# ssheybani/baby-vision-curriculum

Measured on AMD Instinct MI355X. Metric: video clips/sec (node) VideoMAE-base 16x224^2 bf16 pretraining, higher is better.
Workload: dtype bf16

## Files before the change

### __graft_entry__.py

```python
import importlib.util
import os
import subprocess
import sys

ROOT = os.path.dirname(os.path.abspath(__file__))
PKG_DIR = os.path.join(ROOT, "baby-vision-curriculum_amd")
CSRC = os.path.join(PKG_DIR, "csrc")
LIB = os.path.join(PKG_DIR, "libbvc_hip.so")
PRODUCT_SOURCES = ["gemm.hip", "gemm_persist.hip", "gemm8.hip", "gemm_as.hip", "attention.hip", "rowops.hip", "stack.hip", "videomae.hip", "jepa.hip", "comm.hip"]
EXPERIMENT_SOURCES = [os.path.join("experiments", "gemm_big.hip"), os.path.join("experiments", "gemm_pp.hip")]
EXPERIMENT_INCLUDES = [os.path.join("experiments", "attention_dq_wave96.inc")]
HEADERS = ["common.h", "gemm.h", "gemm_tile.h", "attention.h", "rowops.h", "stack.h", os.path.join("..", "..", "include", "bvc.h")]


def _experiments():
    return "BVC_EXPERIMENTS" in os.environ.get("BVC_EXTRA_HIPCC_FLAGS", "")


def _sources():
    return PRODUCT_SOURCES + (EXPERIMENT_SOURCES if _experiments() else [])


SOURCES = PRODUCT_SOURCES


EXPERIMENT_FLAGS = {"attention.hip": ["-mllvm", "-amdgpu-mfma-vgpr-form=1"]}


def _extra_flags(src):
    return EXPERIMENT_FLAGS.get(src, []) if _experiments() else []


HASH_FILE = LIB + ".srchash"


def _source_hash():
    import hashlib
    h = hashlib.sha256()
    for f in _sources() + HEADERS + (EXPERIMENT_INCLUDES if _experiments() else []):
        with open(os.path.join(CSRC, f), "rb") as fh:
            h.update(f.encode() + b"\0" + fh.read())
    h.update(os.environ.get("BVC_EXTRA_HIPCC_FLAGS", "").encode())
    return h.hexdigest()


def _stale():
    if not (os.path.exists(LIB) and os.path.exists(HASH_FILE)):
        return True
    with open(HASH_FILE) as fh:
        return fh.read().strip() != _source_hash()


def _hash_of(files):
# ... 98 lines not shown
```

### baby-vision-curriculum_amd/_lib.py

```python
import ctypes
import os

_HERE = os.path.dirname(os.path.abspath(__file__))
LIB_PATH = os.environ.get("BVC_LIB_PATH") or os.path.join(_HERE, "libbvc_hip.so")

c_void_p, c_int, c_int64, c_float, c_char_p = ctypes.c_void_p, ctypes.c_int, ctypes.c_int64, ctypes.c_float, ctypes.c_char_p
c_double = ctypes.c_double


class BvcError(RuntimeError):
    pass


class VideoMAEConfigC(ctypes.Structure):
    _fields_ = [(n, c_int) for n in (
        "image_size", "patch_size", "num_channels", "num_frames", "tubelet_size",
        "hidden_size", "num_hidden_layers", "num_attention_heads", "intermediate_size",
        "decoder_hidden_size", "decoder_num_hidden_layers", "decoder_num_attention_heads",
        "decoder_intermediate_size")] + [("layer_norm_eps", c_float), ("decoder_norm_eps", c_float),
                                         ("norm_pix_loss", c_int)]


class VitConfigC(ctypes.Structure):
    _fields_ = [(n, c_int) for n in ("image_size", "patch_size", "num_channels", "num_frames", "tubelet_size", "embed_dim",
# ... 110 lines not shown
    "bvc_op_gemm_plan_dw": (c_int, [ctypes.POINTER(GemmDesc), c_int]),
    "bvc_op_attention_fwd": (c_int, [c_void_p, c_void_p, c_void_p, c_int, c_int, c_int, c_int, c_void_p]),
    "bvc_op_attention_bwd": (c_int, [c_void_p, c_void_p, c_void_p, c_void_p, c_void_p, c_void_p, c_int, c_int, c_int, c_int, c_void_p]),
    "bvc_op_attention_bwd_part": (c_int, [c_void_p, c_void_p, c_void_p, c_void_p, c_void_p, c_void_p, c_int, c_int, c_int, c_int, c_int, c_void_p]),
    "bvc_op_layernorm_fwd": (c_int, [c_void_p, c_int, c_int, c_int, c_void_p, c_void_p, c_void_p, c_void_p, c_void_p,
                                     c_int, c_int, c_float, c_void_p]),
    "bvc_op_layernorm_bwd": (c_int, [c_void_p, c_void_p, c_int, c_int, c_int, c_void_p, c_void_p, c_void_p, c_void_p,
                                     c_int, c_void_p, c_void_p, c_void_p, c_void_p, c_int, c_int, c_void_p]),
    "bvc_op_layernorm_bwd_workspace": (c_int64, [c_int, c_int]),
    "bvc_op_colsum_bf16": (c_int, [c_void_p, c_int, c_int, c_int, c_float, c_void_p, c_void_p, c_void_p]),
    "bvc_op_cast_bf16": (c_int, [c_void_p, c_void_p, c_int64, c_void_p]),
    "bvc_op_row_normalize": (c_int, [c_void_p, c_void_p, c_void_p, c_int, c_int, c_float, c_void_p]),
    "bvc_op_row_normalize_bwd": (c_int, [c_void_p, c_void_p, c_void_p, c_void_p, c_int, c_int, c_void_p]),
    "bvc_op_nce_finalize": (c_int, [c_void_p, c_int, c_float, c_int64, c_void_p, c_void_p, c_void_p]),
    "bvc_op_sgd_step": (c_int, [c_void_p, c_void_p, c_void_p, c_int64, c_float, c_float, c_float, c_float, c_int, c_int, c_int,
                                c_void_p, c_void_p, c_int, c_void_p, c_void_p]),
    "bvc_videomae_shadow": (c_int, [c_void_p, c_int, ctypes.POINTER(c_void_p), ctypes.POINTER(c_int64)]),
    "bvc_vit_shadow": (c_int, [c_void_p, c_int, ctypes.POINTER(c_void_p), ctypes.POINTER(c_int64)]),
    "bvc_predictor_shadow": (c_int, [c_void_p, c_int, ctypes.POINTER(c_void_p), ctypes.POINTER(c_int64)]),
    "bvc_op_adam_prepare": (c_int, [c_void_p, c_double, c_double, c_double, c_void_p, c_void_p]),
    "bvc_op_adam_step": (c_int, [c_void_p, c_void_p, c_void_p, c_void_p, c_int64, c_double, c_double, c_double, c_double, c_double,
                                 c_int, c_int, c_void_p, c_void_p, c_void_p, c_int, c_void_p, c_void_p]),
    "bvc_op_row_ln_selected": (c_int, [c_int, c_int, c_int, c_int]),
    "bvc_op_sgd_step_segments": (c_int, [c_void_p, c_void_p, c_void_p, c_int64, c_void_p, c_void_p, c_void_p, c_int, c_void_p, c_void_p, c_void_p,
                                         c_int, c_void_p, c_void_p]),
    "bvc_op_adam_step_segments": (c_int, [c_void_p, c_void_p, c_void_p, c_void_p, c_int64, c_void_p, c_void_p, c_void_p, c_int, c_void_p, c_void_p,
                                          c_void_p, c_void_p, c_void_p, c_int, c_void_p, c_void_p]),
    "bvc_op_nonfinite_check": (c_int, [c_void_p, c_int64, c_void_p, c_void_p]),
    "bvc_op_mask_index": (c_int, [c_void_p, c_int, c_int, c_int, c_int, c_void_p, c_void_p, c_void_p, c_void_p]),
    "bvc_op_gather_patches": (c_int, [c_void_p, c_void_p, c_void_p, c_int, c_int, c_int, c_int, c_int, c_int, c_int, c_int, c_void_p]),
    "bvc_op_pixel_labels": (c_int, [c_void_p, c_void_p, c_void_p, c_int, c_int, c_int, c_int, c_int, c_int, c_int, c_int, c_int, c_void_p]),
    "bvc_comm_unique_id": (c_int, [c_void_p]),
    "bvc_comm_init": (c_int, [c_int, c_int, c_void_p, ctypes.POINTER(c_void_p)]),
    "bvc_comm_destroy": (c_int, [c_void_p]),
    "bvc_comm_stream": (c_void_p, [c_void_p]),
    "bvc_comm_rank": (c_int, [c_void_p]),
    "bvc_comm_world": (c_int, [c_void_p]),
    "bvc_comm_library": (c_char_p, []),
    "bvc_allreduce_bucket": (c_int, [c_void_p, c_void_p, c_int64, c_int, c_void_p]),
    "bvc_comm_wait": (c_int, [c_void_p, c_void_p]),
    "bvc_allgather": (c_int, [c_void_p, c_void_p, c_void_p, c_int64, c_void_p]),
    "bvc_allreduce": (c_int, [c_void_p, c_void_p, c_int64, c_int, c_void_p]),
    "bvc_broadcast": (c_int, [c_void_p, c_void_p, c_int64, c_int, c_void_p]),
}

_lib = None
# ... 33 lines not shown
```

### baby-vision-curriculum_amd/csrc/attention.h

```cpp
#pragma once
#include "common.h"

namespace bvc {
int launch_attn_fwd(const bf16_t* qkv, bf16_t* ctx, float* lse, int B, int N, int H, int head_dim, hipStream_t stream,
                    float softmax_scale = 0.f);
int launch_attn_bwd(const bf16_t* qkv, const bf16_t* ctx, const bf16_t* dctx, const float* lse, float* delta,
                    bf16_t* dqkv, int B, int N, int H, int head_dim, hipStream_t stream, float softmax_scale = 0.f, int parts = 3);
}
```

### baby-vision-curriculum_amd/csrc/attention.hip

```cpp
#include <stdlib.h>

#include "attention.h"

namespace bvc {

#define AS3 __attribute__((address_space(3)))
#define MFMA32(a, b, c) __builtin_amdgcn_mfma_f32_32x32x16_bf16((a), (b), (c), 0, 0, 0)

template <int HD>
__device__ __forceinline__ int swz_dual(int r) {
    if constexpr (HD == 64) return (((r >> 1) & 1) << 2) | ((r >> 2) & 3);
    else return (r >> 2) & 3;
}

template <int HD, int NW = 4>
__device__ __forceinline__ void stage64(__amdgpu_buffer_rsrc_t rs, int row0, int ld, int col0, char* lds,
                                        int wave, int lane) {
    constexpr int CPR = HD / 8;
    constexpr int RPP = 64 / CPR;
#pragma unroll
    for (int jj = 0; jj < (HD / 8 + NW - 1) / NW; ++jj) {
        const int j = wave + NW * jj;
        if (NW > HD / 8 && j >= HD / 8) break;
        const int r = RPP * j + lane / CPR;
        const int c = (lane % CPR) ^ swz_dual<HD>(r);
// ... 115 lines not shown
        s[r] = fast_exp2(fmaf(s[r], scale_log2, nm));
        rs += s[r];
    }
    st.l_run += rs;
    const bf16x8 p0 = acc_to_frag(s, 0), p1 = acc_to_frag(s, 1);
#pragma unroll
    for (int t = 0; t < HD / 32; ++t) st.o[t] = MFMA32(lds_tr<VOFF>(lds, fa.tr[t][0], fa.tr[t][1]), p0, st.o[t]);
#pragma unroll
    for (int t = 0; t < HD / 32; ++t) st.o[t] = MFMA32(lds_tr<VOFF + KS>(lds, fa.tr[t][0], fa.tr[t][1]), p1, st.o[t]);
}

__device__ __forceinline__ void attn_block(int tiles, int remap, int& tile, int& bh) {
    const int nb = gridDim.x, bid = blockIdx.x;
    int lid = bid;
    if (remap) {
        const int xq = nb >> 3, xr = nb & 7, xcd = bid & 7;
        lid = (xcd < xr ? xcd * (xq + 1) : xr * (xq + 1) + (xcd - xr) * xq) + (bid >> 3);
    }
    bh = lid / tiles;
    tile = lid - bh * tiles;
}

struct TailSplit { int gs, own, part, valid; };
template <int NW = 4>
__device__ __forceinline__ TailSplit tail_split(int N, int tile, int wave) {
    if constexpr (NW != 4) { TailSplit t; t.valid = NW; t.gs = 1; t.own = wave; t.part = 0; return t; }
    const int rows = N - tile * 128;
    TailSplit t;
    t.valid = rows >= 128 ? 4 : (rows + 31) >> 5;
    t.gs = t.valid == 1 ? 4 : t.valid == 2 ? 2 : 1;
    t.own = t.gs == 1 ? wave : wave & (t.valid - 1);
    t.part = t.gs == 1 ? 0 : wave >> (t.valid - 1);
    return t;
}
template <int NT>
__device__ __forceinline__ void tail_reduce(char* buf, const TailSplit& ts, int lane, f32x16 (&acc)[NT]) {
    AS3 float* cl = (AS3 float*)buf;
    constexpr int SLOT = NT * 16 * 64;
    __syncthreads();
    if (ts.part > 0) {
        AS3 float* w = cl + ((ts.part - 1) * ts.valid + ts.own) * SLOT + lane;
#pragma unroll
        for (int t = 0; t < NT; ++t)
#pragma unroll
            for (int r = 0; r < 16; ++r) w[(t * 16 + r) * 64] = acc[t][r];
    }
    __syncthreads();
    if (ts.part == 0) {
        for (int p = 1; p < ts.gs; ++p) {
            const AS3 float* w = cl + ((p - 1) * ts.valid + ts.own) * SLOT + lane;
#pragma unroll
            for (int t = 0; t < NT; ++t)
// ... 200 lines not shown
        if (kt + 2 < nkt) issue(kt + 2, 0);
        if (mine(2 * kt + 2)) dq_subtile<HD, STG, STG + IMG>(lds, fa, qf, dof, dq, kt * 64 + 64, N, h, scale_log2, nlse, ndel);
        if (kt * 64 + 96 < N && mine(2 * kt + 3))
            dq_subtile<HD, STG + SUB, STG + IMG + SUB>(lds, fa, qf, dof, dq, kt * 64 + 96, N, h, scale_log2, nlse, ndel);
    }
    if (ts.gs > 1) tail_reduce<HD / 32>(smem, ts, lane, dq);
    if (qi < N && ts.part == 0) {
        bf16_t* orow = dqkv + (size_t)(b * N + qi) * ld + head * HD;
#pragma unroll
        for (int t = 0; t < HD / 32; ++t)
#pragma unroll
            for (int g = 0; g < 4; ++g) {
                const int d = 32 * t + 8 * g + 4 * h;
                uint2 a = {pack2bf(dq[t][4 * g] * scale, dq[t][4 * g + 1] * scale), pack2bf(dq[t][4 * g + 2] * scale, dq[t][4 * g + 3] * scale)};
                *reinterpret_cast<uint2*>(orow + d) = a;
            }
    }
}

#ifdef BVC_EXPERIMENTS
#include "experiments/attention_dq_wave96.inc"
#endif

template <int HD, int QOFF, int STAT>
__device__ __forceinline__ void dkdv_subtile(const AS3 char* lds, const FragAddr<HD>& fa, const bf16x8 (&kf)[HD / 16],
                                             const bf16x8 (&vf)[HD / 16], f32x16 (&dk)[HD / 32], f32x16 (&dv)[HD / 32], int q0,
                                             int N, int h, float scale_log2) {
    constexpr int IMG = 64 * HD * 2, KS = 16 * HD * 2;
    constexpr int DOFF = QOFF + IMG;
#ifndef BVC_ATTN_STATS_LDS
    bf16x8 sfrag, one_s, one_d;
    {
        const AS3 float* st = reinterpret_cast<const AS3 float*>(lds + STAT);
        const int r = threadIdx.x & 31;
        const float xl = -st[r] * (1.0f / scale_log2), xd = st[64 + r];
        const uint32_t hh = pack2bf(xl, xd);
        const float lhi = __uint_as_float(hh << 16), dhi = __uint_as_float(hh & 0xffff0000u);
        const uint32_t ll = pack2bf(xl - lhi, xd - dhi);
        union { bf16x8 v; uint32_t u[4]; } f, a, b;
        f.u[0] = h ? 0u : ((hh & 0xffffu) | (ll << 16));
        f.u[1] = h ? 0u : ((hh >> 16) | (ll & 0xffff0000u));
        f.u[2] = 0u; f.u[3] = 0u;
        a.u[0] = h ? 0u : 0x3f803f80u; a.u[1] = 0u; a.u[2] = 0u; a.u[3] = 0u;
        b.u[0] = 0u; b.u[1] = h ? 0u : 0x3f803f80u; b.u[2] = 0u; b.u[3] = 0u;
        sfrag = f.v; one_s = a.v; one_d = b.v;
    }
    f32x16 s = zero16(), dp = zero16();
#pragma unroll
    for (int stp = 0; stp < HD / 16; ++stp) {
        s = MFMA32(lds_rows<QOFF>(lds, fa.rows[stp]), kf[stp], s);
        dp = MFMA32(lds_rows<DOFF>(lds, fa.rows[stp]), vf[stp], dp);
    }
    s = MFMA32(sfrag, one_s, s);
    dp = MFMA32(sfrag, one_d, dp);
#pragma unroll
    for (int r = 0; r < 16; ++r) {
        const float p = fast_exp2(s[r] * scale_log2);
        s[r] = p;
        dp[r] = p * dp[r];
    }
#else
    const AS3 float* stl = reinterpret_cast<const AS3 float*>(lds + STAT) + 4 * h;
    f32x16 s = zero16(), dp;
#pragma unroll
    for (int g = 0; g < 4; ++g) {
        const f32x4 nd = *reinterpret_cast<const AS3 f32x4*>(stl + 64 + 8 * g);
#pragma unroll
        for (int e = 0; e < 4; ++e) dp[4 * g + e] = nd[e];
    }
// ... 98 lines not shown
        if (mine(2 * qt + 2)) dkdv_subtile<HD, STG, STG + 2 * IMG>(lds, fa, kf, vf, dk, dv, qt * 64 + 64, N, h, scale_log2);
        if (qt * 64 + 96 < N && mine(2 * qt + 3)) dkdv_subtile<HD, STG + SUB, STG + 2 * IMG + 128>(lds, fa, kf, vf, dk, dv, qt * 64 + 96, N, h, scale_log2);
    }
    if (ts.gs > 1) {
        tail_reduce<HD / 32>(smem, ts, lane, dk);
        tail_reduce<HD / 32>(smem, ts, lane, dv);
    }
    if (ki < N && ts.part == 0) {
        bf16_t* krow = dqkv + (size_t)(b * N + ki) * ld + D + head * HD;
        bf16_t* vrow = krow + D;
#pragma unroll
        for (int t = 0; t < HD / 32; ++t)
#pragma unroll
            for (int g = 0; g < 4; ++g) {
                const int d = 32 * t + 8 * g + 4 * h;
                uint2 a = {pack2bf(dk[t][4 * g] * scale, dk[t][4 * g + 1] * scale), pack2bf(dk[t][4 * g + 2] * scale, dk[t][4 * g + 3] * scale)};
                *reinterpret_cast<uint2*>(krow + d) = a;
                uint2 e = {pack2bf(dv[t][4 * g], dv[t][4 * g + 1]), pack2bf(dv[t][4 * g + 2], dv[t][4 * g + 3])};
                *reinterpret_cast<uint2*>(vrow + d) = e;
            }
    }
}

template <int HD, int NBT>
__global__ __launch_bounds__(320, 1) void attn_bwd_head_kernel(const bf16_t* __restrict__ qkv, const bf16_t* __restrict__ dctx,
                                                               const bf16_t* __restrict__ ctx, const float* __restrict__ lse,
                                                               bf16_t* __restrict__ dqkv, int N, int H, int D, int nheads,
                                                               uint32_t qkv_bytes, uint32_t dctx_bytes, float scale, float scale_log2) {
    static_assert(HD == 64, "whole-head backward: head_dim 64");
    extern __shared__ __attribute__((aligned(16))) char smem[];
    constexpr int IMG = 192 * HD * 2, SUB = 32 * HD * 2, KS = 16 * HD * 2;
    constexpr int QI = 0, KI = IMG, VI = 2 * IMG, OI = 3 * IMG;
    constexpr int STAT = 4 * IMG;
    constexpr int DST = STAT + 2 * 192 * 4;
    const AS3 char* lds = (const AS3 char*)smem;
    const int tid = threadIdx.x, lane = tid & 63;
    const int wave = __builtin_amdgcn_readfirstlane(tid >> 6);
    const int ld = 3 * D, h = lane >> 5;
    const int NB = NBT > 0 ? NBT : (N + 31) >> 5;
    const __amdgpu_buffer_rsrc_t rq = make_rsrc(qkv, qkv_bytes), rd = make_rsrc(dctx, dctx_bytes);
    const FragAddr<HD> fa = make_frag_addr<HD>(lane);
    const FragAddr<32> fs = make_frag_addr<32>(lane);

    auto stage_qvo = [&](int bh) __attribute__((always_inline)) {
        if (wave < 4) {
            const int b = bh / H, head = bh % H, row0 = b * N;
// ... 173 lines not shown
        }
    }
    __syncthreads();
    if (nxt < nheads) stage_k(nxt);
    }
}

static int xcd_remap() {
#ifdef BVC_EXPERIMENTS
    return getenv("BVC_ATTN_PLAIN_GRID") == nullptr;
#else
    return 1;
#endif
}

static bool head_kernel_enabled() {
#ifdef BVC_EXPERIMENTS
    return getenv("BVC_ATTN_NO_HEAD_KERNEL") == nullptr;
#else
    return true;
#endif
}

template <int HD>
static int fwd_hd(const bf16_t* qkv, bf16_t* ctx, float* lse, int B, int N, int H, hipStream_t stream, float sm_scale) {
    const int D = H * HD;
    const size_t bytes = (size_t)B * N * 3 * D * 2;
    const float scale_log2 = (sm_scale > 0.f ? sm_scale : 1.0f / sqrtf((float)HD)) * 1.4426950408889634f;
#ifdef BVC_EXPERIMENTS
    if (getenv("BVC_ATTN_NW8") != nullptr) {
        const dim3 grid8((unsigned)(((N + 255) / 256) * B * H));
        hipLaunchKernelGGL((attn_fwd_kernel<HD, 8>), grid8, dim3(512), 4 * 64 * HD * 2, stream, qkv, ctx, lse, N, H, D, (uint32_t)bytes, scale_log2,
                           xcd_remap());
        BVC_CHECK_HIP(hipGetLastError());
        return BVC_OK;
    }
#endif
    const dim3 grid((unsigned)(((N + 127) / 128) * B * H));
    hipLaunchKernelGGL((attn_fwd_kernel<HD, 4>), grid, dim3(256), 4 * 64 * HD * 2, stream, qkv, ctx, lse, N, H, D, (uint32_t)bytes, scale_log2,
                       xcd_remap());
    BVC_CHECK_HIP(hipGetLastError());
    return BVC_OK;
}

template <int HD>
static int bwd_hd(const bf16_t* qkv, const bf16_t* ctx, const bf16_t* dctx, const float* lse, float* delta, bf16_t* dqkv, int B,
// ... 26 lines not shown
            const dim3 g((unsigned)(nheads < ncu ? nheads : ncu));
            if (N > 128)
                hipLaunchKernelGGL((attn_bwd_head_kernel<HD, 5>), g, dim3(320), lds, stream, qkv, dctx, ctx, lse, dqkv, N, H, D, nheads,
                                   (uint32_t)bytes, (uint32_t)((size_t)B * N * D * 2), scale, scale_log2);
            else
                hipLaunchKernelGGL((attn_bwd_head_kernel<HD, 0>), g, dim3(320), lds, stream, qkv, dctx, ctx, lse, dqkv, N, H, D, nheads,
                                   (uint32_t)bytes, (uint32_t)((size_t)B * N * D * 2), scale, scale_log2);
            BVC_CHECK_HIP(hipGetLastError());
            return BVC_OK;
        }
    }
    if (parts & 1) {
#ifdef BVC_EXPERIMENTS
    if (getenv("BVC_ATTN_DQ_W") != nullptr) {
        constexpr int NB = 3;
        const dim3 gridw((unsigned)(((N + 32 * NB - 1) / (32 * NB)) * B * H));
        hipLaunchKernelGGL((attn_bwd_dq_w_kernel<HD, NB>), gridw, dim3(64), kRing * 2 * 32 * HD * 2, stream, qkv, dctx, ctx, lse, delta, dqkv, N, H, D,
                           (uint32_t)bytes, scale, scale_log2, remap);
    } else
#endif
    hipLaunchKernelGGL(attn_bwd_dq_kernel<HD>, grid, dim3(256), 4 * 64 * HD * 2, stream, qkv, dctx, ctx, lse, delta, dqkv, N, H, D,
                       (uint32_t)bytes, scale, scale_log2, remap);
    }
    if (parts & 2)
    hipLaunchKernelGGL(attn_bwd_dkdv_kernel<HD>, grid, dim3(256), 2 * (2 * 64 * HD * 2 + 512), stream, qkv, dctx, lse, delta, dqkv, N, H, D,
                       (uint32_t)bytes, (uint32_t)((size_t)B * N * D * 2), (uint32_t)((size_t)B * H * N * 4), scale, scale_log2, remap);
    BVC_CHECK_HIP(hipGetLastError());
    return BVC_OK;
}

int launch_attn_fwd(const bf16_t* qkv, bf16_t* ctx, float* lse, int B, int N, int H, int head_dim, hipStream_t stream, float sm_scale) {
    BVC_REQUIRE(B > 0 && N > 0 && H > 0, "attn_fwd: empty shape");
    BVC_REQUIRE(head_dim == 64 || head_dim == 32, "attn_fwd: head_dim %d unsupported (32 or 64)", head_dim);
    BVC_REQUIRE((size_t)B * N * 3 * H * head_dim * 2 < 0xffffffffull, "attn_fwd: qkv larger than 4 GiB");
    return head_dim == 64 ? fwd_hd<64>(qkv, ctx, lse, B, N, H, stream, sm_scale) : fwd_hd<32>(qkv, ctx, lse, B, N, H, stream, sm_scale);
}

int launch_attn_bwd(const bf16_t* qkv, const bf16_t* ctx, const bf16_t* dctx, const float* lse, float* delta,
                    bf16_t* dqkv, int B, int N, int H, int head_dim, hipStream_t stream, float sm_scale, int parts) {
    BVC_REQUIRE(B > 0 && N > 0 && H > 0, "attn_bwd: empty shape");
    BVC_REQUIRE(head_dim == 64 || head_dim == 32, "attn_bwd: head_dim %d unsupported (32 or 64)", head_dim);
    BVC_REQUIRE((size_t)B * N * 3 * H * head_dim * 2 < 0xffffffffull, "attn_bwd: qkv larger than 4 GiB");
    return head_dim == 64 ? bwd_hd<64>(qkv, ctx, dctx, lse, delta, dqkv, B, N, H, stream, sm_scale, parts)
                          : bwd_hd<32>(qkv, ctx, dctx, lse, delta, dqkv, B, N, H, stream, sm_scale, parts);
}

}
```

### baby-vision-curriculum_amd/csrc/gemm.h

```cpp
#pragma once
#include "common.h"
#include "../../include/bvc.h"

namespace bvc {

enum GemmLayout { GEMM_NT = BVC_GEMM_NT, GEMM_NN = BVC_GEMM_NN, GEMM_TN = BVC_GEMM_TN };

enum GemmEpilogue {
    EPI_F32 = BVC_EPI_F32,
    EPI_BF16 = BVC_EPI_BF16,
    EPI_GELU = BVC_EPI_GELU,
    EPI_RESID = BVC_EPI_RESID,
    EPI_POS = BVC_EPI_POS,
    EPI_E2D = BVC_EPI_E2D,
    EPI_LOSS = BVC_EPI_LOSS,
    EPI_DGELU = BVC_EPI_DGELU,
    EPI_F32_BF16 = BVC_EPI_F32_BF16,
    EPI_RELU = BVC_EPI_RELU,
    EPI_DRELU = BVC_EPI_DRELU,
    EPI_NCE = BVC_EPI_NCE,
    EPI_NCE_BWD = BVC_EPI_NCE_BWD,
    EPI_RESID_LN = BVC_EPI_RESID_LN,
    EPI_DLN = BVC_EPI_DLN
};

using GemmProblem = bvc_gemm_desc;

constexpr int kMaxGroup = 4;

struct Options { int gemm8 = 0; int dw_overlap = 0; int row_ln = 0; int row_stagger = 1; };
Options& options();

struct DryRun { bool on = false; char name[160] = ""; };
DryRun& dry_run();

int launch_gemm(const GemmProblem* probs, int nprob, GemmLayout layout, int tile_cfg, hipStream_t stream, int stages = -1);

int gemm_num_tiles(const GemmProblem& p, int tile_cfg);
int gemm_pick_tile(const GemmProblem* probs, int nprob, int tile_cfg);
bool gemm_row_ln_ok(int M, int N, int K);
constexpr size_t kRowLnPartFloats = 512 * 2 * 384;

}
```

### baby-vision-curriculum_amd/csrc/videomae.hip

```cpp
#include <math.h>
#include <stdarg.h>
#include <stdio.h>
#include <stdlib.h>
#include <string.h>

#include <algorithm>
#include <string>
#include <vector>

#include "stack.h"

namespace bvc {
static thread_local char g_err[1024] = "";
void set_error(const char* fmt, ...) {
    va_list ap;
    va_start(ap, fmt);
    vsnprintf(g_err, sizeof(g_err), fmt, ap);
    va_end(ap);
}
const char* last_error() { return g_err; }
}

using namespace bvc;

// ... 88 lines not shown
        px.is_u8 = 1;
        for (int c = 0; c < 4; ++c) {
            BVC_REQUIRE(fmt->std[c] != 0.f || c >= channels, "pixel format: std[%d] is zero", c);
            px.mean[c] = fmt->mean[c];
            px.stdv[c] = c < channels ? fmt->std[c] : 1.f;
        }
    }
    *out = px;
    return BVC_OK;
}
}

extern "C" {

const char* bvc_last_error(void) { return bvc::last_error(); }
const char* bvc_version(void) { return "gfx950;bvc-hip-r5"; }

int bvc_set_option(const char* name, int value) {
    BVC_REQUIRE(name != nullptr, "set_option: null name");
    if (!strcmp(name, "gemm8")) { BVC_REQUIRE(value >= -1 && value <= 1, "set_option: gemm8 takes -1 / 0 / 1"); options().gemm8 = value; }
    else if (!strcmp(name, "dw_overlap")) options().dw_overlap = value != 0;
    else if (!strcmp(name, "row_stagger")) options().row_stagger = value != 0;
    else if (!strcmp(name, "row_ln")) { BVC_REQUIRE(value >= -1 && value <= 1, "set_option: row_ln takes -1 / 0 / 1"); options().row_ln = value; }
    else BVC_REQUIRE(false, "set_option: unknown option '%s'", name);
    return BVC_OK;
}
int bvc_get_option(const char* name) {
    if (name && !strcmp(name, "gemm8")) return options().gemm8;
    if (name && !strcmp(name, "dw_overlap")) return options().dw_overlap;
    if (name && !strcmp(name, "row_ln")) return options().row_ln;
    if (name && !strcmp(name, "row_stagger")) return options().row_stagger;
    bvc::set_error("get_option: unknown option '%s'", name ? name : "(null)");
    return BVC_ERR_INVALID;
}

int bvc_videomae_param_count(const bvc_videomae_config* cfg) {
    if (!cfg || check_config(*cfg) != BVC_OK) return BVC_ERR_INVALID;
    return (int)make_layout(*cfg).entries.size();
}

int64_t bvc_videomae_param_numel(const bvc_videomae_config* cfg) {
    if (!cfg || check_config(*cfg) != BVC_OK) return BVC_ERR_INVALID;
    return make_layout(*cfg).total;
}

int bvc_videomae_param_info(const bvc_videomae_config* cfg, int index, char* name, int name_cap, int64_t* offset,
                            int64_t* numel, int* ndim, int64_t shape[5]) {
    BVC_REQUIRE(cfg && name && offset && numel && ndim && shape, "param_info: null argument");
    TRY(check_config(*cfg));
    const Layout L = make_layout(*cfg);
    BVC_REQUIRE(index >= 0 && index < (int)L.entries.size(), "param_info: index %d out of range", index);
    const ParamEntry& e = L.entries[index];
    snprintf(name, name_cap, "%s", e.name.c_str());
    *offset = e.offset; *numel = e.numel; *ndim = e.ndim;
// ... 341 lines not shown
    const int rc = launch_gemm(problems, count, (GemmLayout)layout, tile_cfg, nullptr, stages);
    d.on = false;
    if (rc == BVC_OK) snprintf(name, name_cap, "%s", d.name);
    return rc;
}
int bvc_op_gemm_plan_dw(bvc_gemm_desc* problems, int count) {
    BVC_REQUIRE(problems && count >= 1 && count <= 4, "op_gemm_plan_dw: bad argument");
    return plan_dw(problems, count);
}
int bvc_op_gemm_num_tiles(const bvc_gemm_desc* problem, int tile_cfg) {
    if (!problem) return BVC_ERR_INVALID;
    return gemm_num_tiles(*problem, tile_cfg);
}
int bvc_op_attention_fwd(const void* qkv, void* ctx_out, float* lse, int B, int N, int H, int head_dim, void* stream) {
    BVC_REQUIRE(qkv && ctx_out && lse, "op_attention_fwd: null argument");
    return launch_attn_fwd((const bf16_t*)qkv, (bf16_t*)ctx_out, lse, B, N, H, head_dim, (hipStream_t)stream);
}
int bvc_op_attention_bwd(const void* qkv, const void* ctx_in, const void* dctx, const float* lse, float* delta, void* dqkv,
                         int B, int N, int H, int head_dim, void* stream) {
    BVC_REQUIRE(qkv && ctx_in && dctx && lse && delta && dqkv, "op_attention_bwd: null argument");
    return launch_attn_bwd((const bf16_t*)qkv, (const bf16_t*)ctx_in, (const bf16_t*)dctx, lse, delta, (bf16_t*)dqkv, B, N, H, head_dim,
                           (hipStream_t)stream);
}
int bvc_op_attention_bwd_part(const void* qkv, const void* ctx_in, const void* dctx, const float* lse, float* delta, void* dqkv,
                              int B, int N, int H, int head_dim, int part, void* stream) {
    BVC_REQUIRE(qkv && ctx_in && dctx && lse && delta && dqkv, "op_attention_bwd_part: null argument");
    BVC_REQUIRE(part == 1 || part == 2, "op_attention_bwd_part: part is 1 (dQ + delta) or 2 (dK, dV)");
    return launch_attn_bwd((const bf16_t*)qkv, (const bf16_t*)ctx_in, (const bf16_t*)dctx, lse, delta, (bf16_t*)dqkv, B, N, H, head_dim,
                           (hipStream_t)stream, 0.f, part);
}
int bvc_op_layernorm_fwd(const float* x, int rin, int rout, int roff, const float* gamma, const float* beta, void* y,
                         float* mean, float* rstd, int M, int D, float eps, void* stream) {
    BVC_REQUIRE(x && gamma && beta && y && mean && rstd, "op_layernorm_fwd: null argument");
    return launch_ln_fwd(x, RowMap{rin, rout, roff}, gamma, beta, (bf16_t*)y, mean, rstd, M, D, eps, (hipStream_t)stream);
}
int bvc_op_layernorm_bwd(const void* dy, const float* x, int rin, int rout, int roff, const float* mean, const float* rstd,
                         const float* gamma, float* dres, int accumulate, void* dres_bf16, float* dgamma, float* dbeta,
                         float* workspace, int M, int D, void* stream) {
    BVC_REQUIRE(dy && x && mean && rstd && gamma && dres && dgamma && dbeta && workspace, "op_layernorm_bwd: null argument");
    return launch_ln_bwd((const bf16_t*)dy, x, RowMap{rin, rout, roff}, mean, rstd, gamma, dres, accumulate, (bf16_t*)dres_bf16,
                         dgamma, dbeta, workspace, M, D, (hipStream_t)stream);
}
int64_t bvc_op_layernorm_bwd_workspace(int M, int D) { return (int64_t)ln_bwd_workspace_floats(M, D); }
int bvc_op_colsum_bf16(const void* X, int M, int N, int ld, float alpha, const float* alpha_dev, float* out, void* stream) {
    BVC_REQUIRE(X && out, "op_colsum_bf16: null argument");
    return launch_colsum_bf16_scaled((const bf16_t*)X, M, N, ld, alpha, alpha_dev, out, (hipStream_t)stream);
// ... 85 lines not shown
```

### baby-vision-curriculum_amd/probe.py

```python
import ctypes

import torch

from . import _lib, _ops

PEAK_BF16_TFLOPS = 2500.0
PEAK_HBM_GBS = 8000.0


def _time(fn, iters=5, warm=2):
    for _ in range(warm):
        fn()
    e0, e1 = torch.cuda.Event(enable_timing=True), torch.cuda.Event(enable_timing=True)
    e0.record()
    for _ in range(iters):
        fn()
    e1.record()
    torch.cuda.synchronize()
    return e0.elapsed_time(e1) * 1e3 / iters


def _rb(dev, *shape):
    return torch.randn(*shape, device=dev, dtype=torch.bfloat16)

# ... 117 lines not shown


def _attention_rows(dev, B, add):
    lib = _lib.lib()
    st = _lib.current_stream_ptr
    for label, N, H, count in (("enc", 160, 12, 12), ("dec", 1568, 6, 4)):
        Dm = 64 * H
        qkv, ctx, dctx, dqkv = _rb(dev, B * N, 3 * Dm), _rb(dev, B * N, Dm), _rb(dev, B * N, Dm), _rb(dev, B * N, 3 * Dm)
        lse = torch.empty(B * H * N, device=dev)
        delta = torch.empty(B * H * N, device=dev)
        p = lambda t: ctypes.c_void_p(t.data_ptr())
        fwd = lambda: _lib.check(lib.bvc_op_attention_fwd(p(qkv), p(ctx), p(lse), B, N, H, 64, st()), "attention_fwd")
        dq = lambda: _lib.check(lib.bvc_op_attention_bwd_part(p(qkv), p(ctx), p(dctx), p(lse), p(delta), p(dqkv), B, N, H, 64, 1, st()), "attention_bwd dq")
        dkv = lambda: _lib.check(lib.bvc_op_attention_bwd_part(p(qkv), p(ctx), p(dctx), p(lse), p(delta), p(dqkv), B, N, H, 64, 2, st()), "attention_bwd dkdv")
        unit = 2.0 * N * N * 64 * H * B
        tok = 2.0 * B * N * Dm
        add("bvc::attn_fwd_kernel<64>", f"{label} attention fwd", count, _time(fwd), 2 * unit, 4 * tok)
        if N <= 160:
            bwd = lambda: _lib.check(lib.bvc_op_attention_bwd(p(qkv), p(ctx), p(dctx), p(lse), p(delta), p(dqkv), B, N, H, 64, st()), "attention_bwd")
            add(f"bvc::attn_bwd_head_kernel<64, {5 if N > 128 else 0}>", f"{label} attention bwd (whole head: S, dP, dV, dK, dQ)", count, _time(bwd),
                5 * unit, 8 * tok)
            continue
        add("bvc::attn_bwd_dq_kernel<64>", f"{label} attention bwd dQ (S, dP, dQ)", count, _time(dq), 3 * unit, 6 * tok)
        add("bvc::attn_bwd_dkdv_kernel<64>", f"{label} attention bwd dK dV (recomputes S, dP)", count, _time(dkv), 2 * unit, 6 * tok)


def _layernorm_rows(dev, B, add):
    lib = _lib.lib()
    st = _lib.current_stream_ptr
    p = lambda t: ctypes.c_void_p(t.data_ptr())
    fused = bool(lib.bvc_op_row_ln_selected(B * 1568, 384, 1536, 6))
    for label, M, Dm, count, count_bwd in (("enc", B * 160, 768, 24, 24), ("dec", B * 1568, 384, 1 if fused else 8, 0 if fused else 8),
                                           ("final", B * 1408, 384, 1, 1)):
        x, dres = torch.randn(M, Dm, device=dev), torch.randn(M, Dm, device=dev)
        gmm, bta = torch.ones(Dm, device=dev), torch.zeros(Dm, device=dev)
        y, dy, dresb = _rb(dev, M, Dm), _rb(dev, M, Dm), _rb(dev, M, Dm)
        mean, rstd = torch.empty(M, device=dev), torch.empty(M, device=dev)
        dg, db = torch.zeros(Dm, device=dev), torch.zeros(Dm, device=dev)
        ws = torch.empty(int(lib.bvc_op_layernorm_bwd_workspace(M, Dm)), device=dev)
        fwd = lambda: _lib.check(lib.bvc_op_layernorm_fwd(p(x), 0, 0, 0, p(gmm), p(bta), p(y), p(mean), p(rstd), M, Dm, 1e-12, st()), "layernorm_fwd")
        bwd = lambda: _lib.check(lib.bvc_op_layernorm_bwd(p(dy), p(x), 0, 0, 0, p(mean), p(rstd), p(gmm), p(dres), 1, p(dresb), p(dg), p(db),
                                                          p(ws), M, Dm, st()), "layernorm_bwd")
        e = float(M) * Dm
        add("bvc::ln_fwd_kernel", f"{label} LayerNorm fwd", count, _time(fwd), 0.0, 6 * e)
        if count_bwd:
            add("bvc::ln_bwd_kernel (+ ln_param_reduce)", f"{label} LayerNorm bwd", count_bwd, _time(bwd), 0.0, 16 * e)

# ... 33 lines not shown
```

### include/bvc.h

```cpp
#ifndef BVC_H
#define BVC_H

#include <stddef.h>
#include <stdint.h>

#ifdef __cplusplus
extern "C" {
#endif

#define BVC_OK 0
#define BVC_ERR_INVALID (-1)
#define BVC_ERR_HIP (-2)
#define BVC_ERR_STATE (-3)

const char* bvc_last_error(void);
const char* bvc_version(void);
int bvc_set_option(const char* name, int value);
int bvc_get_option(const char* name);

typedef struct bvc_videomae_config {
    int image_size, patch_size, num_channels, num_frames, tubelet_size;
    int hidden_size, num_hidden_layers, num_attention_heads, intermediate_size;
    int decoder_hidden_size, decoder_num_hidden_layers, decoder_num_attention_heads, decoder_intermediate_size;
    float layer_norm_eps;
// ... 102 lines not shown
    float alpha;
    const float* alpha_dev;
    int epi, split_k;
    void* C; int ldc; void* C2;
    const float* bias; const float* resid; const void* aux; int ldaux;
    const int* rowtok; const float* pos; const float* labels; float* partial;
    int rin, rout;
    float* rowsum;
    const float* ln_gamma; const float* ln_beta;
    float* ln_mean; float* ln_rstd;
    float ln_eps;
    const float* ln_x;
    float* ln_part; float* ln_dgamma; float* ln_dbeta;
} bvc_gemm_desc;
int bvc_op_gemm(const bvc_gemm_desc* problems, int count, int layout, int tile_cfg, int stages, void* stream);
int bvc_op_gemm_num_tiles(const bvc_gemm_desc* problem, int tile_cfg);
int bvc_op_gemm_kernel(const bvc_gemm_desc* problems, int count, int layout, int tile_cfg, int stages, char* name, int name_cap);
int bvc_op_row_ln_selected(int tokens, int width, int mlp_width, int heads);
int bvc_op_gemm_plan_dw(bvc_gemm_desc* problems, int count);

int bvc_op_attention_fwd(const void* qkv, void* ctx_out, float* lse, int B, int N, int H, int head_dim, void* stream);
int bvc_op_attention_bwd(const void* qkv, const void* ctx_in, const void* dctx, const float* lse, float* delta_scratch,
                         void* dqkv, int B, int N, int H, int head_dim, void* stream);
int bvc_op_attention_bwd_part(const void* qkv, const void* ctx_in, const void* dctx, const float* lse, float* delta_scratch,
                              void* dqkv, int B, int N, int H, int head_dim, int part, void* stream);
int bvc_op_layernorm_fwd(const float* x, int rin, int rout, int roff, const float* gamma, const float* beta, void* y_bf16,
                         float* mean, float* rstd, int M, int D, float eps, void* stream);
int bvc_op_layernorm_bwd(const void* dy_bf16, const float* x, int rin, int rout, int roff, const float* mean,
                         const float* rstd, const float* gamma, float* dres, int accumulate, void* dres_bf16,
                         float* dgamma, float* dbeta, float* workspace, int M, int D, void* stream);
int64_t bvc_op_layernorm_bwd_workspace(int M, int D);
int bvc_op_colsum_bf16(const void* X, int M, int N, int ld, float alpha, const float* alpha_dev, float* out, void* stream);
int bvc_op_cast_bf16(const float* in, void* out, int64_t n, void* stream);
int bvc_op_row_normalize(const float* f, void* fn_bf16, float* inv_norm, int n, int p, float eps, void* stream);
int bvc_op_row_normalize_bwd(const float* f, const float* inv_norm, const float* dfn, float* df, int n, int p, void* stream);
int bvc_op_nce_finalize(const float* partial, int ntiles, float inv_temperature, int64_t npos, float* loss, float* stats, void* stream);
int bvc_op_sgd_step(float* params, float* grads, float* momentum_buf, int64_t n, float lr, float momentum, float dampening,
                    float weight_decay, int nesterov, int first_step, int maximize, const float* grad_scale,
                    const float* found_inf, int write_unscaled_grads, void* bf16_shadow, void* stream);
int bvc_op_adam_prepare(float* state3, double lr, double beta1, double beta2, const float* found_inf, void* stream);
int bvc_op_adam_step(float* params, float* grads, float* exp_avg, float* exp_avg_sq, int64_t n, double lr, double beta1, double beta2,
                     double eps, double weight_decay, int decoupled, int maximize, const float* state3, const float* grad_scale,
                     const float* found_inf, int write_unscaled_grads, void* bf16_shadow, void* stream);
#define BVC_OPT_MAX_GROUPS 8
typedef struct bvc_sgd_groups {
    int ngroups;
// ... 42 lines not shown
```

Before: 3235.

## Add opt-in 64-keys-per-wave dK/dV attention backward kernel and always apply MFMA VGPR flag

Adds an attention backward dK/dV kernel where each wave owns 64 keys, with AGPR-resident accumulators and a three-stage LDS pipeline. It is selected only when the new attn_dkdv option is set, and is meant to raise reuse of staged Q/dO tiles per key. Separately, the MFMA VGPR-form compiler flag for attention.hip is now always applied rather than only in experiment builds. That changes register allocation for all default attention kernels and could help or hurt occupancy and scheduling.

```diff
diff --git a/__graft_entry__.py b/__graft_entry__.py
--- a/__graft_entry__.py
+++ b/__graft_entry__.py
@@ -24,11 +24,11 @@
 SOURCES = PRODUCT_SOURCES
 
 
-EXPERIMENT_FLAGS = {"attention.hip": ["-mllvm", "-amdgpu-mfma-vgpr-form=1"]}
+SOURCE_FLAGS = {"attention.hip": ["-mllvm", "-amdgpu-mfma-vgpr-form=1"]}
 
 
 def _extra_flags(src):
-    return EXPERIMENT_FLAGS.get(src, []) if _experiments() else []
+    return SOURCE_FLAGS.get(src, [])
 
 
 HASH_FILE = LIB + ".srchash"
diff --git a/baby-vision-curriculum_amd/_lib.py b/baby-vision-curriculum_amd/_lib.py
--- a/baby-vision-curriculum_amd/_lib.py
+++ b/baby-vision-curriculum_amd/_lib.py
@@ -156,6 +156,7 @@
     "bvc_op_adam_step": (c_int, [c_void_p, c_void_p, c_void_p, c_void_p, c_int64, c_double, c_double, c_double, c_double, c_double,
                                  c_int, c_int, c_void_p, c_void_p, c_void_p, c_int, c_void_p, c_void_p]),
     "bvc_op_row_ln_selected": (c_int, [c_int, c_int, c_int, c_int]),
+    "bvc_op_attention_dkdv_selected": (c_int, [c_int, c_int]),
     "bvc_op_sgd_step_segments": (c_int, [c_void_p, c_void_p, c_void_p, c_int64, c_void_p, c_void_p, c_void_p, c_int, c_void_p, c_void_p, c_void_p,
                                          c_int, c_void_p, c_void_p]),
     "bvc_op_adam_step_segments": (c_int, [c_void_p, c_void_p, c_void_p, c_void_p, c_int64, c_void_p, c_void_p, c_void_p, c_int, c_void_p, c_void_p,
diff --git a/baby-vision-curriculum_amd/csrc/attention.h b/baby-vision-curriculum_amd/csrc/attention.h
--- a/baby-vision-curriculum_amd/csrc/attention.h
+++ b/baby-vision-curriculum_amd/csrc/attention.h
@@ -6,4 +6,5 @@
                     float softmax_scale = 0.f);
 int launch_attn_bwd(const bf16_t* qkv, const bf16_t* ctx, const bf16_t* dctx, const float* lse, float* delta,
                     bf16_t* dqkv, int B, int N, int H, int head_dim, hipStream_t stream, float softmax_scale = 0.f, int parts = 3);
+int attn_dkdv_kernel(int N, int head_dim);
 }
diff --git a/baby-vision-curriculum_amd/csrc/attention.hip b/baby-vision-curriculum_amd/csrc/attention.hip
--- a/baby-vision-curriculum_amd/csrc/attention.hip
+++ b/baby-vision-curriculum_amd/csrc/attention.hip
@@ -1,6 +1,9 @@
 #include <stdlib.h>
 
+#include <type_traits>
+
 #include "attention.h"
+#include "gemm.h"
 
 namespace bvc {
 
@@ -162,12 +165,13 @@
 }
 
 struct TailSplit { int gs, own, part, valid; };
-template <int NW = 4>
+template <int NW = 4, int RW = 32>
 __device__ __forceinline__ TailSplit tail_split(int N, int tile, int wave) {
     if constexpr (NW != 4) { TailSplit t; t.valid = NW; t.gs = 1; t.own = wave; t.part = 0; return t; }
-    const int rows = N - tile * 128;
+    constexpr int LG = RW == 64 ? 6 : 5;
+    const int rows = N - tile * 4 * RW;
     TailSplit t;
-    t.valid = rows >= 128 ? 4 : (rows + 31) >> 5;
+    t.valid = rows >= 4 * RW ? 4 : (rows + RW - 1) >> LG;
     t.gs = t.valid == 1 ? 4 : t.valid == 2 ? 2 : 1;
     t.own = t.gs == 1 ? wave : wave & (t.valid - 1);
     t.part = t.gs == 1 ? 0 : wave >> (t.valid - 1);
@@ -414,6 +418,22 @@
 #include "experiments/attention_dq_wave96.inc"
 #endif
 
+__device__ __forceinline__ void dkdv_stat_frags(const AS3 char* stat, int h, float scale_log2, bf16x8& sfrag, bf16x8& one_s, bf16x8& one_d) {
+    const AS3 float* st = reinterpret_cast<const AS3 float*>(stat);
+    const int r = threadIdx.x & 31;
+    const float xl = -st[r] * (1.0f / scale_log2), xd = st[64 + r];
+    const uint32_t hh = pack2bf(xl, xd);
+    const float lhi = __uint_as_float(hh << 16), dhi = __uint_as_float(hh & 0xffff0000u);
+    const uint32_t ll = pack2bf(xl - lhi, xd - dhi);
+    union { bf16x8 v; uint32_t u[4]; } f, a, b;
+    f.u[0] = h ? 0u : ((hh & 0xffffu) | (ll << 16));
+    f.u[1] = h ? 0u : ((hh >> 16) | (ll & 0xffff0000u));
+    f.u[2] = 0u; f.u[3] = 0u;
+    a.u[0] = h ? 0u : 0x3f803f80u; a.u[1] = 0u; a.u[2] = 0u; a.u[3] = 0u;
+    b.u[0] = 0u; b.u[1] = h ? 0u : 0x3f803f80u; b.u[2] = 0u; b.u[3] = 0u;
+    sfrag = f.v; one_s = a.v; one_d = b.v;
+}
+
 template <int HD, int QOFF, int STAT>
 __device__ __forceinline__ void dkdv_subtile(const AS3 char* lds, const FragAddr<HD>& fa, const bf16x8 (&kf)[HD / 16],
                                              const bf16x8 (&vf)[HD / 16], f32x16 (&dk)[HD / 32], f32x16 (&dv)[HD / 32], int q0,
@@ -422,21 +442,7 @@
     constexpr int DOFF = QOFF + IMG;
 #ifndef BVC_ATTN_STATS_LDS
     bf16x8 sfrag, one_s, one_d;
-    {
-        const AS3 float* st = reinterpret_cast<const AS3 float*>(lds + STAT);
-        const int r = threadIdx.x & 31;
-        const float xl = -st[r] * (1.0f / scale_log2), xd = st[64 + r];
-        const uint32_t hh = pack2bf(xl, xd);
-        const float lhi = __uint_as_float(hh << 16), dhi = __uint_as_float(hh & 0xffff0000u);
-        const uint32_t ll = pack2bf(xl - lhi, xd - dhi);
-        union { bf16x8 v; uint32_t u[4]; } f, a, b;
-        f.u[0] = h ? 0u : ((hh & 0xffffu) | (ll << 16));
-        f.u[1] = h ? 0u : ((hh >> 16) | (ll & 0xffff0000u));
-        f.u[2] = 0u; f.u[3] = 0u;
-        a.u[0] = h ? 0u : 0x3f803f80u; a.u[1] = 0u; a.u[2] = 0u; a.u[3] = 0u;
-        b.u[0] = 0u; b.u[1] = h ? 0u : 0x3f803f80u; b.u[2] = 0u; b.u[3] = 0u;
-        sfrag = f.v; one_s = a.v; one_d = b.v;
-    }
+    dkdv_stat_frags(lds + STAT, h, scale_log2, sfrag, one_s, one_d);
     f32x16 s = zero16(), dp = zero16();
 #pragma unroll
     for (int stp = 0; stp < HD / 16; ++stp) {
@@ -581,6 +587,181 @@
     }
 }
 
+__device__ __forceinline__ void mfma_agpr(f32x16& acc, const bf16x8& a, const bf16x8& b) {
+    asm volatile("s_nop 1\n\tv_mfma_f32_32x32x16_bf16 %0, %1, %2, %0" : "+a"(acc) : "v"(a), "v"(b));
+}
+__device__ __forceinline__ void agpr_drain() { asm volatile("s_nop 15\n\ts_nop 7" ::: "memory"); }
+
+template <int HD, int NK, int QOFF, int STAT>
+__device__ __forceinline__ void dkdv_w64_subtile(const AS3 char* lds, const FragAddr<HD>& fa, const bf16x8 (&kf)[2][HD / 16],
+                                                 const bf16x8 (&vf)[2][HD / 16], f32x16 (&dk)[2 * HD / 32], f32x16 (&dv)[2 * HD / 32],
+                                                 int q0, int N, int h, float scale_log2) {
+    constexpr int IMG = 64 * HD * 2, KS = 16 * HD * 2, NT = HD / 32;
+    constexpr int DOFF = QOFF + IMG;
+    bf16x8 sfrag, one_s, one_d;
+    dkdv_stat_frags(lds + STAT, h, scale_log2, sfrag, one_s, one_d);
+    f32x16 s[NK], dp[NK];
+#pragma unroll
+    for (int k = 0; k < NK; ++k) { s[k] = zero16(); dp[k] = zero16(); }
+#pragma unroll
+    for (int stp = 0; stp < HD / 16; ++stp) {
+        const bf16x8 qr = lds_rows<QOFF>(lds, fa.rows[stp]);
+        const bf16x8 dr = lds_rows<DOFF>(lds, fa.rows[stp]);
+#pragma unroll
+        for (int k = 0; k < NK; ++k) {
+            s[k] = MFMA32(qr, kf[k][stp], s[k]);
+            dp[k] = MFMA32(dr, vf[k][stp], dp[k]);
+        }
+    }
+#pragma unroll
+    for (int k = 0; k < NK; ++k) {
+        s[k] = MFMA32(sfrag, one_s, s[k]);
+        dp[k] = MFMA32(sfrag, one_d, dp[k]);
+    }
+#pragma unroll
+    for (int k = 0; k < NK; ++k)
+#pragma unroll
+        for (int r = 0; r < 16; ++r) {
+            const float p = fast_exp2(s[k][r] * scale_log2);
+            s[k][r] = p;
+            dp[k][r] = p * dp[k][r];
+        }
+    if (q0 + 32 > N) {
+        asm volatile("" ::: "memory");
+#pragma unroll
+        for (int k = 0; k < NK; ++k)
+#pragma unroll
+            for (int r = 0; r < 16; ++r)
+                if (q0 + acc_row(r, h) >= N) { s[k][r] = 0.f; dp[k][r] = 0.f; }
+    }
+    bf16x8 pf[NK][2], df[NK][2];
+#pragma unroll
+    for (int k = 0; k < NK; ++k)
+#pragma unroll
+        for (int j = 0; j < 2; ++j) { pf[k][j] = acc_to_frag(s[k], j); df[k][j] = acc_to_frag(dp[k], j); }
+#pragma unroll
+    for (int j = 0; j < 2; ++j)
+#pragma unroll
+        for (int t = 0; t < NT; ++t) {
+            const bf16x8 ot = lds_tr<DOFF>(lds + j * KS, fa.tr[t][0], fa.tr[t][1]);
+            const bf16x8 qt = lds_tr<QOFF>(lds + j * KS, fa.tr[t][0], fa.tr[t][1]);
+#pragma unroll
+            for (int k = 0; k < NK; ++k) {
+                mfma_agpr(dv[NT * k + t], ot, pf[k][j]);
+                mfma_agpr(dk[NT * k + t], qt, df[k][j]);
+            }
+        }
+}
+
+template <int HD>
+__global__ __launch_bounds__(256, 1) void attn_bwd_dkdv_w64_kernel(const bf16_t* __restrict__ qkv, const bf16_t* __restrict__ dctx,
+                                                                   const float* __restrict__ lse, const float* __restrict__ delta,
+                                                                   bf16_t* __restrict__ dqkv, int N, int H, int D,
+                                                                   uint32_t qkv_bytes, uint32_t dctx_bytes, uint32_t stat_bytes,
+                                                                   float scale, float scale_log2, int remap) {
+    static_assert(HD == 64, "64 keys per wave: head_dim 64");
+    extern __shared__ __attribute__((aligned(16))) char smem[];
+    constexpr int IMG = 64 * HD * 2, SUB = 32 * HD * 2, STG = 2 * IMG + 512, NT = HD / 32;
+    const AS3 char* lds = (const AS3 char*)smem;
+    const int tid = threadIdx.x, lane = tid & 63;
+    const int wave = __builtin_amdgcn_readfirstlane(tid >> 6);
+    int tile_, bh;
+    attn_block((N + 255) >> 8, remap, tile_, bh);
+    const int b = bh / H, head = bh % H;
+    const int ld = 3 * D;
+    const TailSplit ts = tail_split<4, 64>(N, tile_, wave);
+    const int key0 = tile_ * 256 + ts.own * 64;
+    const bool two = key0 + 32 < N;
+    const int h = lane >> 5;
+    const int gm = ts.gs - 1;
+    auto mine = [&](int sub) { return (sub & gm) == ts.part; };
+    const __amdgpu_buffer_rsrc_t rq = make_rsrc(qkv, qkv_bytes);
+    const __amdgpu_buffer_rsrc_t rd = make_rsrc(dctx, dctx_bytes);
+    const __amdgpu_buffer_rsrc_t rl = make_rsrc(lse, stat_bytes);
+    const __amdgpu_buffer_rsrc_t re = make_rsrc(delta, stat_bytes);
+    const FragAddr<HD> fa = make_frag_addr<HD>(lane);
+
+    bf16x8 kf[2][HD / 16], vf[2][HD / 16];
+#pragma unroll
+    for (int k = 0; k < 2; ++k) {
+        const int kc = min(key0 + 32 * k + (lane & 31), N - 1);
+        const bf16_t* krow = qkv + (size_t)(b * N + kc) * ld + D + head * HD + 8 * h;
+#pragma unroll
+        for (int st = 0; st < HD / 16; ++st) { kf[k][st] = load8(krow + 16 * st); vf[k][st] = load8(krow + D + 16 * st); }
+    }
+#pragma unroll
+    for (int k = 0; k < 2; ++k)
+#pragma unroll
+        for (int stq = 0; stq < HD / 16; ++stq) { settle(kf[k][stq]); settle(vf[k][stq]); }
+    f32x16 dk[2 * NT], dv[2 * NT];
+#pragma unroll
+    for (int i = 0; i < 2 * NT; ++i) {
+        dk[i] = zero16(); dv[i] = zero16();
+        asm volatile("" : "+a"(dk[i]), "+a"(dv[i]));
+    }
+
+    const int nqt = (N + 63) >> 6;
+    const int qrow0 = b * N;
+    auto issue = [&](int qt, int stage) {
+        char* dst = smem + stage * STG;
+        stage64<HD>(rq, qrow0 + qt * 64, ld, head * HD, dst, wave, lane);
+        stage64<HD>(rd, qrow0 + qt * 64, D, head * HD, dst + IMG, wave, lane);
+        if (wave == 0)
+            glds4(rl, (uint32_t)(((size_t)bh * N + qt * 64 + lane) * 4), (uint32_t)(size_t)((AS3 char*)dst) + 2 * IMG);
+        if (wave == 1)
+            glds4(re, (uint32_t)(((size_t)bh * N + qt * 64 + lane) * 4), (uint32_t)(size_t)((AS3 char*)dst) + 2 * IMG + 256);
+    };
+    auto query_loop = [&](auto nk) __attribute__((always_inline)) {
+        constexpr int NK = decltype(nk)::value;
+        issue(0, 0);
+        if (nqt > 1) issue(1, 1);
+        int stage = 0;
+        for (int qt = 0; qt < nqt; ++qt) {
+            if (qt + 1 < nqt) {
+                if (wave < 2) asm volatile("s_waitcnt vmcnt(5)" ::: "memory");
+                else asm volatile("s_waitcnt vmcnt(4)" ::: "memory");
+            } else {
+                asm volatile("s_waitcnt vmcnt(0)" ::: "memory");
+            }
+            __syncthreads();
+            if (qt + 2 < nqt) issue(qt + 2, stage == 0 ? 2 : stage - 1);
+            const AS3 char* base = lds + stage * STG;
+            const int q0 = qt * 64;
+            if (mine(2 * qt)) dkdv_w64_subtile<HD, NK, 0, 2 * IMG>(base, fa, kf, vf, dk, dv, q0, N, h, scale_log2);
+            if (q0 + 32 < N && mine(2 * qt + 1)) dkdv_w64_subtile<HD, NK, SUB, 2 * IMG + 128>(base, fa, kf, vf, dk, dv, q0 + 32, N, h, scale_log2);
+            stage = stage == 2 ? 0 : stage + 1;
+        }
+    };
+    if (two) query_loop(std::integral_constant<int, 2>{});
+    else query_loop(std::integral_constant<int, 1>{});
+    agpr_drain();
+    if (ts.gs > 1) {
+        tail_reduce<2 * NT>(smem, ts, lane, dk);
+        tail_reduce<2 * NT>(smem, ts, lane, dv);
+    }
+    if (ts.part == 0) {
+#pragma unroll
+        for (int k = 0; k < 2; ++k) {
+            const int ki = key0 + 32 * k + (lane & 31);
+            if (ki >= N) continue;
+            bf16_t* krow = dqkv + (size_t)(b * N + ki) * ld + D + head * HD;
+            bf16_t* vrow = krow + D;
+#pragma unroll
+            for (int t = 0; t < NT; ++t)
+#pragma unroll
+                for (int g = 0; g < 4; ++g) {
+                    const f32x16& a_ = dk[NT * k + t];
+                    const f32x16& e_ = dv[NT * k + t];
+                    const int d = 32 * t + 8 * g + 4 * h;
+                    uint2 a = {pack2bf(a_[4 * g] * scale, a_[4 * g + 1] * scale), pack2bf(a_[4 * g + 2] * scale, a_[4 * g + 3] * scale)};
+                    *reinterpret_cast<uint2*>(krow + d) = a;
+                    uint2 e = {pack2bf(e_[4 * g], e_[4 * g + 1]), pack2bf(e_[4 * g + 2], e_[4 * g + 3])};
+                    *reinterpret_cast<uint2*>(vrow + d) = e;
+                }
+        }
+    }
+}
+
 template <int HD, int NBT>
 __global__ __launch_bounds__(320, 1) void attn_bwd_head_kernel(const bf16_t* __restrict__ qkv, const bf16_t* __restrict__ dctx,
                                                                const bf16_t* __restrict__ ctx, const float* __restrict__ lse,
@@ -800,6 +981,8 @@
 #endif
 }
 
+static bool attn_dkdv_w64() { return options().attn_dkdv > 0; }
+
 template <int HD>
 static int fwd_hd(const bf16_t* qkv, bf16_t* ctx, float* lse, int B, int N, int H, hipStream_t stream, float sm_scale) {
     const int D = H * HD;
@@ -872,9 +1055,17 @@
     hipLaunchKernelGGL(attn_bwd_dq_kernel<HD>, grid, dim3(256), 4 * 64 * HD * 2, stream, qkv, dctx, ctx, lse, delta, dqkv, N, H, D,
                        (uint32_t)bytes, scale, scale_log2, remap);
     }
-    if (parts & 2)
-    hipLaunchKernelGGL(attn_bwd_dkdv_kernel<HD>, grid, dim3(256), 2 * (2 * 64 * HD * 2 + 512), stream, qkv, dctx, lse, delta, dqkv, N, H, D,
-                       (uint32_t)bytes, (uint32_t)((size_t)B * N * D * 2), (uint32_t)((size_t)B * H * N * 4), scale, scale_log2, remap);
+    if (parts & 2) {
+        if (HD == 64 && attn_dkdv_w64()) {
+            const dim3 grid64((unsigned)(((N + 255) / 256) * B * H));
+            hipLaunchKernelGGL(attn_bwd_dkdv_w64_kernel<64>, grid64, dim3(256), 3 * (2 * 64 * HD * 2 + 512), stream, qkv, dctx, lse, delta, dqkv,
+                               N, H, D, (uint32_t)bytes, (uint32_t)((size_t)B * N * D * 2), (uint32_t)((size_t)B * H * N * 4), scale, scale_log2,
+                               remap);
+        } else {
+            hipLaunchKernelGGL(attn_bwd_dkdv_kernel<HD>, grid, dim3(256), 2 * (2 * 64 * HD * 2 + 512), stream, qkv, dctx, lse, delta, dqkv, N, H, D,
+                               (uint32_t)bytes, (uint32_t)((size_t)B * N * D * 2), (uint32_t)((size_t)B * H * N * 4), scale, scale_log2, remap);
+        }
+    }
     BVC_CHECK_HIP(hipGetLastError());
     return BVC_OK;
 }
@@ -895,4 +1086,6 @@
                           : bwd_hd<32>(qkv, ctx, dctx, lse, delta, dqkv, B, N, H, stream, sm_scale, parts);
 }
 
-}
+int attn_dkdv_kernel(int N, int head_dim) { return head_dim == 64 && N > 0 && attn_dkdv_w64() ? 1 : 0; }
+
+}
diff --git a/baby-vision-curriculum_amd/csrc/gemm.h b/baby-vision-curriculum_amd/csrc/gemm.h
--- a/baby-vision-curriculum_amd/csrc/gemm.h
+++ b/baby-vision-curriculum_amd/csrc/gemm.h
@@ -28,7 +28,7 @@
 
 constexpr int kMaxGroup = 4;
 
-struct Options { int gemm8 = 0; int dw_overlap = 0; int row_ln = 0; int row_stagger = 1; };
+struct Options { int gemm8 = 0; int dw_overlap = 0; int row_ln = 0; int row_stagger = 1; int attn_dkdv = 0; };
 Options& options();
 
 struct DryRun { bool on = false; char name[160] = ""; };
diff --git a/baby-vision-curriculum_amd/csrc/videomae.hip b/baby-vision-curriculum_amd/csrc/videomae.hip
--- a/baby-vision-curriculum_amd/csrc/videomae.hip
+++ b/baby-vision-curriculum_amd/csrc/videomae.hip
@@ -134,6 +134,7 @@
     else if (!strcmp(name, "dw_overlap")) options().dw_overlap = value != 0;
     else if (!strcmp(name, "row_stagger")) options().row_stagger = value != 0;
     else if (!strcmp(name, "row_ln")) { BVC_REQUIRE(value >= -1 && value <= 1, "set_option: row_ln takes -1 / 0 / 1"); options().row_ln = value; }
+    else if (!strcmp(name, "attn_dkdv")) { BVC_REQUIRE(value >= -1 && value <= 1, "set_option: attn_dkdv takes -1 / 0 / 1"); options().attn_dkdv = value; }
     else BVC_REQUIRE(false, "set_option: unknown option '%s'", name);
     return BVC_OK;
 }
@@ -142,6 +143,7 @@
     if (name && !strcmp(name, "dw_overlap")) return options().dw_overlap;
     if (name && !strcmp(name, "row_ln")) return options().row_ln;
     if (name && !strcmp(name, "row_stagger")) return options().row_stagger;
+    if (name && !strcmp(name, "attn_dkdv")) return options().attn_dkdv;
     bvc::set_error("get_option: unknown option '%s'", name ? name : "(null)");
     return BVC_ERR_INVALID;
 }
@@ -529,6 +531,7 @@
     return launch_attn_bwd((const bf16_t*)qkv, (const bf16_t*)ctx_in, (const bf16_t*)dctx, lse, delta, (bf16_t*)dqkv, B, N, H, head_dim,
                            (hipStream_t)stream);
 }
+int bvc_op_attention_dkdv_selected(int N, int head_dim) { return attn_dkdv_kernel(N, head_dim); }
 int bvc_op_attention_bwd_part(const void* qkv, const void* ctx_in, const void* dctx, const float* lse, float* delta, void* dqkv,
                               int B, int N, int H, int head_dim, int part, void* stream) {
     BVC_REQUIRE(qkv && ctx_in && dctx && lse && delta && dqkv, "op_attention_bwd_part: null argument");
diff --git a/baby-vision-curriculum_amd/probe.py b/baby-vision-curriculum_amd/probe.py
--- a/baby-vision-curriculum_amd/probe.py
+++ b/baby-vision-curriculum_amd/probe.py
@@ -163,7 +163,8 @@
                 5 * unit, 8 * tok)
             continue
         add("bvc::attn_bwd_dq_kernel<64>", f"{label} attention bwd dQ (S, dP, dQ)", count, _time(dq), 3 * unit, 6 * tok)
-        add("bvc::attn_bwd_dkdv_kernel<64>", f"{label} attention bwd dK dV (recomputes S, dP)", count, _time(dkv), 2 * unit, 6 * tok)
+        dkdv = "attn_bwd_dkdv_w64_kernel" if lib.bvc_op_attention_dkdv_selected(N, 64) else "attn_bwd_dkdv_kernel"
+        add(f"bvc::{dkdv}<64>", f"{label} attention bwd dK dV (recomputes S, dP)", count, _time(dkv), 2 * unit, 6 * tok)
 
 
 def _layernorm_rows(dev, B, add):
diff --git a/include/bvc.h b/include/bvc.h
--- a/include/bvc.h
+++ b/include/bvc.h
@@ -148,6 +148,7 @@
 int bvc_op_attention_fwd(const void* qkv, void* ctx_out, float* lse, int B, int N, int H, int head_dim, void* stream);
 int bvc_op_attention_bwd(const void* qkv, const void* ctx_in, const void* dctx, const float* lse, float* delta_scratch,
                          void* dqkv, int B, int N, int H, int head_dim, void* stream);
+int bvc_op_attention_dkdv_selected(int N, int head_dim);
 int bvc_op_attention_bwd_part(const void* qkv, const void* ctx_in, const void* dctx, const float* lse, float* delta_scratch,
                               void* dqkv, int B, int N, int H, int head_dim, int part, void* stream);
 int bvc_op_layernorm_fwd(const float* x, int rin, int rout, int roff, const float* gamma, const float* beta, void* y_bf16,
```

After: 3230, median of 6. No clear change (-0.1%).
